# lan496/torch-m3gnet

Hardware: AMD Instinct MI355X
Metric: atom-steps/sec (energy+forces) on 10k-atom PBC batch, 1/2/4/8 MI355X (higher is better)
Workload: dtype f32; 1 GPU; single 10000-atom fcc Cu PBC supercell per GPU (10x10x25 cells, a=3.61 A, jitter 0.025 A), r_cut 5 A / 3-body 4 A, default M3GNet (l_max=n_max=3, D=64, 3 blocks), energy+forces+stress; precision=fp32, atoms_per_gpu=10000, edges_per_gpu=420000, triplets_per_gpu=3060000

## Files before the change

torch-m3gnet_amd/csrc/m3g_api.hip:

```cpp
#include <cmath>
#include <cstdarg>
#include <cstdio>
#include <cstdlib>
#include <cstring>

#include "m3g_internal.h"

namespace m3g {

static thread_local char g_err[512] = "";
void set_error(const char* fmt, ...) {
  va_list ap;
  va_start(ap, fmt);
  vsnprintf(g_err, sizeof(g_err), fmt, ap);
  va_end(ap);
}

static inline size_t align_up(size_t x, size_t a = 256) { return (x + a - 1) / a * a; }

static void layout_mlp(MlpW& m, size_t& off) {
  auto take = [&](size_t n) { size_t r = off; off += (n + 63) / 64 * 64; return r; };
  m.w1a_t = take(kDP * 2 * kDP); m.w1b_t = take(kDP * 2 * kDP); m.w1c_t = take(kDP * 2 * kDP);
  m.b1 = take(2 * kDP);
  m.w2d_t = take(kDP * kDP); m.w2g_t = take(kDP * kDP);
// ... 284 lines not shown
  return M3G_OK;
}

extern "C" int m3g_plan_set_const(m3g_plan* plan, const char* name, const float* host_data, int64_t numel) {
  if (!plan || !name || !host_data) { set_error("m3g_plan_set_const: null argument"); return M3G_ERR_VALUE; }
  auto exp = expected_consts(plan->cfg);
  auto it = exp.find(name);
  if (it == exp.end()) { set_error("unknown constant '%s'", name); return M3G_ERR_VALUE; }
  if (it->second != numel) { set_error("constant '%s': expected %lld values, got %lld", name, (long long)it->second, (long long)numel); return M3G_ERR_VALUE; }
  plan->cvals[name].assign(host_data, host_data + numel);
  plan->committed = false;
  return M3G_OK;
}

extern "C" int m3g_plan_set_option(m3g_plan* plan, const char* name, int32_t value) {
  if (!plan || !name) { set_error("m3g_plan_set_option: null argument"); return M3G_ERR_VALUE; }
  if (strcmp(name, "edge_kernel") == 0) {
    if (value < 0 || value > 2) { set_error("edge_kernel must be 0 (VALU baseline), 1 (MFMA) or 2 (any-size path)"); return M3G_ERR_VALUE; }
    if (plan->generic && value != 2) { set_error("this model size only runs on the any-size path (edge_kernel = 2)"); return M3G_ERR_UNSUPPORTED; }
    plan->edge_kernel = value;
    return M3G_OK;
  }
  if (strcmp(name, "precision") == 0) {
    if (value != kPrecF32 && value != kPrecBf16x3 && value != kPrecF16x3) {
      set_error("precision must be 0 (fp32: exact fp32 MFMA products), 1 (bf16x3 split products) or 2 (f16x3: scaled fp16 split products)");
      return M3G_ERR_VALUE;
    }
    plan->precision = value;
    return M3G_OK;
  }
  if (strcmp(name, "save_p1") == 0) {
    plan->save_p1 = value != 0;
    return M3G_OK;
  }
  if (strcmp(name, "save_p2") == 0) {
    plan->save_p2 = value != 0;
    return M3G_OK;
  }
  if (strcmp(name, "rev_kernel") == 0) {
    if (value != 0 && value != 1) { set_error("rev_kernel must be 0 (node-MLP + edge-MLP kernel pair) or 1 (fused)"); return M3G_ERR_VALUE; }
    plan->rev_kernel = value;
    return M3G_OK;
  }
  if (strcmp(name, "small_tiles") == 0) {
    if (value < 0) { set_error("small_tiles must be >= 0"); return M3G_ERR_VALUE; }
    plan->small_tiles = value;
    plan->small_tiles_fwd = value;
    drop_graphs(plan);
    return M3G_OK;
  }
  if (strcmp(name, "small_tiles_fwd") == 0) {
    if (value < 0) { set_error("small_tiles_fwd must be >= 0"); return M3G_ERR_VALUE; }
    plan->small_tiles_fwd = value;
    drop_graphs(plan);
    return M3G_OK;
  }
  if (strcmp(name, "dp1_by_dst") == 0) {
    plan->dp1_by_dst = value != 0;
    drop_graphs(plan);
    return M3G_OK;
  }
  if (strcmp(name, "split_node_tiles") == 0) {
    if (value < 0) { set_error("split_node_tiles must be >= 0"); return M3G_ERR_VALUE; }
    plan->split_node_tiles = value;
    drop_graphs(plan);
    return M3G_OK;
  }
  if (strcmp(name, "fuse_node_tb") == 0) {
    plan->fuse_node_tb = value != 0;
    drop_graphs(plan);
    return M3G_OK;
  }
  if (strcmp(name, "debug_node_tb_polls") == 0) {
    plan->debug_node_tb_polls = value;
    drop_graphs(plan);
    return M3G_OK;
  }
  if (strcmp(name, "split_tail") == 0) {
    if (value < 0 || value > 2) { set_error("split_tail must be 0 (never), 1 (a single left-over tile) or 2 (one or two)"); return M3G_ERR_VALUE; }
    plan->split_tail = value;
    drop_graphs(plan);
    return M3G_OK;
  }
  if (strcmp(name, "small_launches") == 0) {
    plan->small_launches = value != 0;
    drop_graphs(plan);
    return M3G_OK;
  }
  if (strcmp(name, "graph_replay") == 0) {
    plan->graph_replay = value != 0;
    if (!plan->graph_replay) drop_graphs(plan);
    return M3G_OK;
  }
  if (strcmp(name, "overlap") == 0) {
    plan->overlap = value != 0;
    return M3G_OK;
  }
  if (strcmp(name, "threebody_moments") == 0) {
    plan->tb_moments = value != 0;
    return M3G_OK;
  }
  if (strcmp(name, "legendre_backward") == 0) {
    if (value != 0 && value != 1) { set_error("legendre_backward: 0 (exact derivative) or 1 (the reference's backward)"); return M3G_ERR_VALUE; }
    plan->legendre_ref = value != 0;
    drop_graphs(plan);
    return M3G_OK;
  }
  if (strcmp(name, "readout_f16") == 0) {
    plan->readout_f16 = value != 0;
    return M3G_OK;
  }
  if (strcmp(name, "stress_mode") == 0) {
    if (value != 0 && value != 1) { set_error("stress_mode must be 0 (reference: sum pos (x) F / V) or 1 (pair virial)"); return M3G_ERR_VALUE; }
    plan->stress_mode = value;
    return M3G_OK;
  }
  if (strcmp(name, "debug_force_move") == 0) {
    plan->debug_force_move = value != 0;
    plan->committed = false;
    return M3G_OK;
  }
  if (strcmp(name, "stamps") == 0) {
    plan->stamp_target = value == 3 ? 2 : value == 2 ? 1 : 0;
    if (value && !plan->d_stamps) {
      M3G_HIP_CHECK(hipMalloc((void**)&plan->d_stamps, 256 * 16 * 12 * sizeof(unsigned long long)));
      M3G_HIP_CHECK(hipMemset(plan->d_stamps, 0, 256 * 16 * 12 * sizeof(unsigned long long)));
    } else if (!value && plan->d_stamps) {
      (void)hipFree(plan->d_stamps);
      plan->d_stamps = nullptr;
    }
    return M3G_OK;
  }
  set_error("unknown option '%s'", name);
  return M3G_ERR_VALUE;
}

extern "C" int m3g_debug_read_stamps(m3g_plan* plan, uint64_t* host_out ) {
  if (!plan || !host_out || !plan->d_stamps) { set_error("stamps not enabled"); return M3G_ERR_STATE; }
  M3G_HIP_CHECK(hipMemcpy(host_out, plan->d_stamps, 256 * 16 * 12 * sizeof(unsigned long long), hipMemcpyDeviceToHost));
  return M3G_OK;
}

extern "C" int m3g_plan_commit(m3g_plan* plan) {
  if (!plan) { set_error("m3g_plan_commit: null plan"); return M3G_ERR_VALUE; }
  drop_graphs(plan);
  const m3g_config& cfg = plan->cfg;
  for (auto& kv : expected_params(cfg))
    if (!plan->params.count(kv.first)) { set_error("parameter '%s' was never set", kv.first.c_str()); return M3G_ERR_STATE; }
  for (auto& kv : expected_consts(cfg))
    if (!plan->cvals.count(kv.first)) { set_error("constant '%s' was never set", kv.first.c_str()); return M3G_ERR_STATE; }
  const int D = cfg.embedding_dim, R = cfg.n_max, L = cfg.l_max, C = L * R, B = cfg.num_blocks;
  {
    int dev = 0;
    M3G_HIP_CHECK(hipGetDevice(&dev));
    if (plan->device >= 0 && (plan->device != dev || plan->debug_force_move)) {
      M3G_HIP_CHECK(hipSetDevice(plan->device));
      M3G_HIP_CHECK(hipDeviceSynchronize());
      if (plan->d_weights) { (void)hipFree(plan->d_weights); plan->d_weights = nullptr; }
      free_mfma_images(plan);
      generic_free(plan);
      if (plan->d_stamps) { (void)hipFree(plan->d_stamps); plan->d_stamps = nullptr; }
      release_device_handles(plan);
      M3G_HIP_CHECK(hipSetDevice(dev));
      plan->debug_force_move = false;
    }
    M3G_HIP_CHECK(hipDeviceSynchronize());
// ... 52 lines not shown
    put_t(blob, bw.tb_wd_t, kDP, wd, D, C, 0, C); put_t(blob, bw.tb_wg_t, kDP, wg, D, C, 0, C);
    put_n(blob, bw.tb_wd, kCP, wd, D, C, 0, C); put_n(blob, bw.tb_wg, kCP, wg, D, C, 0, C);
    pack_mlp(blob, bw.e, *plan, cv + ".concat_edge_update", cv + ".edge_linear.weight", D, R);
    pack_mlp(blob, bw.n, *plan, cv + ".concat_node_update", cv + ".node_linear.weight", D, R);
  }
  {
    const ReadoutW& r = wl.ro;
    snprintf(buf, sizeof buf, "model.%d.gated", 6 + 2 * B);
    std::string ro = buf;
    const float* wd0 = plan->params.at(ro + ".dense.0.weight").data();
    const float* wg0 = plan->params.at(ro + ".gate.0.weight").data();
    const float* wd2 = plan->params.at(ro + ".dense.2.weight").data();
    const float* wg2 = plan->params.at(ro + ".gate.2.weight").data();
    put_t(blob, r.w1d_t, kDP, wd0, D, D, 0, D); put_t(blob, r.w1g_t, kDP, wg0, D, D, 0, D);
    put_t(blob, r.w2d_t, kDP, wd2, D, D, 0, D); put_t(blob, r.w2g_t, kDP, wg2, D, D, 0, D);
    put_n(blob, r.w1d, kDP, wd0, D, D, 0, D); put_n(blob, r.w1g, kDP, wg0, D, D, 0, D);
    put_n(blob, r.w2d, kDP, wd2, D, D, 0, D); put_n(blob, r.w2g, kDP, wg2, D, D, 0, D);
    for (int o = 0; o < D; ++o) {
      blob[r.b1d + o] = plan->params.at(ro + ".dense.0.bias")[o];
      blob[r.b1g + o] = plan->params.at(ro + ".gate.0.bias")[o];
      blob[r.b2d + o] = plan->params.at(ro + ".dense.2.bias")[o];
      blob[r.b2g + o] = plan->params.at(ro + ".gate.2.bias")[o];
      blob[r.w3d + o] = plan->params.at(ro + ".dense.4.weight")[o];
      blob[r.w3g + o] = plan->params.at(ro + ".gate.4.weight")[o];
    }
    blob[r.b3] = plan->params.at(ro + ".dense.4.bias")[0];
    blob[r.b3 + 1] = plan->params.at(ro + ".gate.4.bias")[0];
  }
  if (!plan->d_weights) M3G_HIP_CHECK(hipMalloc((void**)&plan->d_weights, wl.total * sizeof(float)));
  M3G_HIP_CHECK(hipMemcpy(plan->d_weights, blob.data(), wl.total * sizeof(float), hipMemcpyHostToDevice));
  { int rc = pack_mfma_images(plan); if (rc) return rc; }
  plan->committed = true;
  return M3G_OK;
}

extern "C" int m3g_workspace_bytes(const m3g_plan* plan, int64_t N, int64_t E, int64_t T, int64_t S, size_t* bytes) {
  if (!plan || !bytes || N < 0 || E < 0 || T < 0 || S < 0) { set_error("m3g_workspace_bytes: bad argument"); return M3G_ERR_VALUE; }
  if (plan->edge_kernel == 2) { *bytes = generic_workspace_bytes(plan, N, E, T, S); return M3G_OK; }
  Consts c{};
  c.B = plan->cfg.num_blocks;
  *bytes = work_carve(c, plan->edge_kernel == 1, saved_activations(plan), N, E, T, S, nullptr).total_bytes;
  return M3G_OK;
}

static bool ensure_side_stream(const m3g_plan* plan) {
  if (plan->side_stream) return true;
  if (hipStreamCreateWithFlags(&plan->side_stream, hipStreamNonBlocking) != hipSuccess) { plan->side_stream = nullptr; return false; }
  if (hipEventCreateWithFlags(&plan->ev_fork, hipEventDisableTiming) != hipSuccess ||
      hipEventCreateWithFlags(&plan->ev_join, hipEventDisableTiming) != hipSuccess)
    return false;
  return true;
}

static void drop_graphs(const m3g_plan* plan) {
  for (auto& g : plan->graphs) {
    if (g.exec) (void)hipGraphExecDestroy(g.exec);
    if (g.graph) (void)hipGraphDestroy(g.graph);
  }
  plan->graphs.clear();
}

static int energy_forces_graph(const m3g_plan* plan, const m3g_io* io, void* workspace, size_t workspace_bytes, hipStream_t caller) {
  hipStream_t s = caller;
  const bool via_side = caller == nullptr;
  if (via_side) {
    if (!ensure_side_stream(plan)) { set_error("graph_replay: could not create the internal stream"); return M3G_ERR_HIP; }
    s = plan->side_stream;
    M3G_HIP_CHECK(hipEventRecord(plan->ev_fork, caller));
    M3G_HIP_CHECK(hipStreamWaitEvent(s, plan->ev_fork, 0));
  }
  auto join = [&]() -> int {
    if (via_side) {
      M3G_HIP_CHECK(hipEventRecord(plan->ev_join, s));
      M3G_HIP_CHECK(hipStreamWaitEvent(caller, plan->ev_join, 0));
    }
    return M3G_OK;
  };
  std::vector<unsigned char> key(sizeof(m3g_io) + sizeof(void*) * 2 + sizeof(size_t) + 4 * sizeof(int));
  unsigned char* k = key.data();
  memcpy(k, io, sizeof(m3g_io)); k += sizeof(m3g_io);
  memcpy(k, &workspace, sizeof(void*)); k += sizeof(void*);
  memcpy(k, &s, sizeof(void*)); k += sizeof(void*);
  memcpy(k, &workspace_bytes, sizeof(size_t)); k += sizeof(size_t);
  const int opts[4] = {plan->edge_kernel, plan->rev_kernel + 2 * plan->save_p1 + 4 * plan->save_p2 + 8 * plan->tb_moments + 16 * plan->precision + 64 * plan->readout_f16, plan->stress_mode, plan->overlap};
  memcpy(k, opts, sizeof(opts));
  for (auto& g : plan->graphs)
    if (g.key == key) { M3G_HIP_CHECK(hipGraphLaunch(g.exec, s)); return join(); }
  if (plan->graphs.size() >= 8) drop_graphs(plan);
  m3g_plan::GraphEntry ge;
  ge.key = key;
  M3G_HIP_CHECK(hipStreamBeginCapture(s, hipStreamCaptureModeThreadLocal));
  plan->capturing = true;
  const int rc = m3g_energy_forces(plan, io, workspace, workspace_bytes, (void*)s);
  plan->capturing = false;
  hipError_t e = hipStreamEndCapture(s, &ge.graph);
  if (rc != M3G_OK) { if (ge.graph) (void)hipGraphDestroy(ge.graph); return rc; }
  if (e != hipSuccess || !ge.graph) { set_error("hipStreamEndCapture failed: %s", hipGetErrorString(e)); return M3G_ERR_HIP; }
  e = hipGraphInstantiate(&ge.exec, ge.graph, nullptr, nullptr, 0);
  if (e != hipSuccess) { (void)hipGraphDestroy(ge.graph); set_error("hipGraphInstantiate failed: %s", hipGetErrorString(e)); return M3G_ERR_HIP; }
  plan->graphs.push_back(ge);
  M3G_HIP_CHECK(hipGraphLaunch(ge.exec, s));
  return join();
}

extern "C" int m3g_count_launches(const m3g_plan* plan, const m3g_io* io, void* workspace, size_t workspace_bytes, int32_t* kernel_launches,
                                  int32_t* other_operations) {
  if (!plan || !io || !kernel_launches) { set_error("m3g_count_launches: null argument"); return M3G_ERR_VALUE; }
  if (plan->capturing) { set_error("m3g_count_launches: a capture is in progress"); return M3G_ERR_STATE; }
  hipStream_t s = nullptr;
  M3G_HIP_CHECK(hipStreamCreateWithFlags(&s, hipStreamNonBlocking));
  hipGraph_t graph = nullptr;
  hipError_t e = hipStreamBeginCapture(s, hipStreamCaptureModeThreadLocal);
  if (e != hipSuccess) { (void)hipStreamDestroy(s); set_error("hipStreamBeginCapture failed: %s", hipGetErrorString(e)); return M3G_ERR_HIP; }
  const bool profile = plan->profile;
  plan->capturing = true;
  plan->profile = false;
  const int rc = m3g_energy_forces(plan, io, workspace, workspace_bytes, (void*)s);
  plan->capturing = false;
  plan->profile = profile;
  e = hipStreamEndCapture(s, &graph);
  (void)hipStreamDestroy(s);
  if (rc != M3G_OK) { if (graph) (void)hipGraphDestroy(graph); return rc; }
  if (e != hipSuccess || !graph) { set_error("hipStreamEndCapture failed: %s", hipGetErrorString(e)); return M3G_ERR_HIP; }
  size_t n = 0;
  e = hipGraphGetNodes(graph, nullptr, &n);
  std::vector<hipGraphNode_t> nodes(n);
  if (e == hipSuccess && n) e = hipGraphGetNodes(graph, nodes.data(), &n);
  int kernels = 0, other = 0;
  for (size_t i = 0; e == hipSuccess && i < n; ++i) {
    hipGraphNodeType ty;
    e = hipGraphNodeGetType(nodes[i], &ty);
    if (e != hipSuccess) break;
    if (ty == hipGraphNodeTypeKernel) ++kernels;
    else if (ty != hipGraphNodeTypeEmpty) ++other;
  }
  (void)hipGraphDestroy(graph);
  if (e != hipSuccess) { set_error("m3g_count_launches: reading the captured graph failed: %s", hipGetErrorString(e)); return M3G_ERR_HIP; }
  *kernel_launches = kernels;
  if (other_operations) *other_operations = other;
  return M3G_OK;
}

static int dp1_format(const m3g_plan* plan) {
  if (!fused_reverse(plan)) return kDp1F32;
  if (dp1_rows_by_dst(plan)) return kDp1F32ByDst;
  return plan->precision == kPrecBf16x3 ? kDp1Packed : plan->precision == kPrecF16x3 ? kDp1Fixed : kDp1F32;
}

extern "C" int m3g_energy_forces(const m3g_plan* plan, const m3g_io* io, void* workspace, size_t workspace_bytes,
                                 void* stream_) {
  if (!plan || !io) { set_error("m3g_energy_forces: null argument"); return M3G_ERR_VALUE; }
  if (!plan->committed) { set_error("m3g_energy_forces: plan parameters not committed"); return M3G_ERR_STATE; }
  {
    int dev = -1;
    M3G_HIP_CHECK(hipGetDevice(&dev));
    if (dev != plan->device) {
      set_error("m3g_energy_forces: the plan was committed on device %d but the current device is %d (commit again on this device)", plan->device, dev);
      return M3G_ERR_STATE;
    }
  }
  if (plan->graph_replay && !plan->capturing && !plan->profile && !plan->overlap)
    return energy_forces_graph(plan, io, workspace, workspace_bytes, (hipStream_t)stream_);
  const int64_t N = io->n_atoms, E = io->n_edges, T = io->n_triplets, S = io->n_structs;
  if (N < 0 || E < 0 || T < 0 || S < 0) { set_error("negative size"); return M3G_ERR_VALUE; }
  if (!io->total_energy || !io->topo || (N > 0 && (!io->pos || !io->atom_types)) || (S > 0 && !io->lattice) ||
      (E > 0 && !io->edge_cell_shift)) {
    set_error("m3g_energy_forces: missing required pointer");
// ... 202 lines not shown
```

torch-m3gnet_amd/csrc/m3g_edge_common.h:

```cpp
#pragma once
#include <utility>

#include "m3g_device.h"
#include "m3g_internal.h"
#include "m3g_dual_chain.h"
#include "m3g_dual_f32.h"
#include "m3g_mfma_common.h"

namespace m3g {

constexpr int kFwdLdsFloats = 8 * kTbSteps * 64 + 2 * (8 * 4 * 4 * 64 + 2 * (4 * 4 * 4 * 64) + 2 * 4 * 64 + 4 * 64) + 4 * 64;
constexpr int kRevMlpFloats = 8 * 4 * 4 * 64 + 4 * (4 * 4 * 4 * 64) + 2 * 4 * 64 + 4 * 8 * 4 * 64 + 64 * 4;
constexpr int kRevEdgeFloats = kRevMlpFloats + 8 * kTbSteps * 64 + 8 * 4 * 64;
#ifndef M3G_WAVES_FWD
#define M3G_WAVES_FWD 16
#endif
constexpr int kWaves = M3G_WAVES_FWD;
#ifndef M3G_WAVES_FWD_H
#define M3G_WAVES_FWD_H 12
#endif
template <int PREC>
#ifndef M3G_WAVES_FWD_BF
#define M3G_WAVES_FWD_BF 12
#endif
// ... 329 lines not shown
struct TbIn { float mb[TBS]; };
template <int TBS>
struct TbIn<kPrecF16x3, TBS> { f16x8 hi, lo; float inv; };

template <int PREC, int TBS>
__device__ __forceinline__ TbIn<PREC, TBS> tb_load(const float* __restrict__ m, int arow, int q, float w_inv) {
  TbIn<PREC, TBS> r;
  if constexpr (PREC == kPrecF16x3) {
    f32x4 v[2] = {f32x4{0.f, 0.f, 0.f, 0.f}, f32x4{0.f, 0.f, 0.f, 0.f}};
    if (arow >= 0 && q < 2) {
      const float* row = m + (int64_t)arow * kCP + 8 * q;
      v[0] = *(const f32x4*)row;
      v[1] = *(const f32x4*)(row + 4);
    }
    const EdgeScale sc = edge_scale<2>(v);
    split8h(v[0], v[1], sc.s, r.hi, r.lo);
    r.inv = sc.inv * w_inv;
  } else {
    static_for<TBS>([&]<int s>() { r.mb[s] = arow >= 0 ? m[(int64_t)arow * kCP + 4 * s + q] : 0.f; });
  }
  return r;
}
template <int PREC, int TBS>
__device__ __forceinline__ void tb_preact_p(const float* tbimg, const TbIn<PREC, TBS>& in, f32x4 (&p)[8], int lane) {
  if constexpr (PREC == kPrecF16x3) {
    const f16x8* hi = reinterpret_cast<const f16x8*>(tbimg) + (lane & 31);
    const f16x8* lo = hi + 8 * 32;
    f16x8 ah = hi[0], al = lo[0];
    static_for<8>([&]<int ob>() {
      f16x8 nh = ah, nl = al;
      if constexpr (ob + 1 < 8) { nh = hi[(ob + 1) * 32]; nl = lo[(ob + 1) * 32]; }
#ifndef M3G_NO_FWD_CHAIN_PREFETCH
      __builtin_amdgcn_sched_barrier(0);
#endif
      f32x4 t = {0.f, 0.f, 0.f, 0.f};
      t = mfma_f16(ah, in.hi, t);
      t = mfma_f16(ah, in.lo, t);
      t = mfma_f16(al, in.hi, t);
      p[ob] = t * in.inv;
#ifndef M3G_NO_FWD_CHAIN_PREFETCH
      __builtin_amdgcn_sched_barrier(0);
#endif
      ah = nh; al = nl;
    });
  } else {
    tb_preact<TBS>(tbimg, in.mb, p, lane);
  }
}

__device__ __forceinline__ void gather_tables(const float* __restrict__ TA, const float* __restrict__ TB, int mlp, int64_t ci,
                                              int64_t cj, int qd, f32x4 (&p1)[8]) {
#ifdef M3G_DIAG_NO_GATHER
  static_for<8>([&]<int ob>() { p1[ob] = f32x4{0.1f, 0.2f, 0.3f, 0.4f}; });
  return;
#endif
  const float* ta = TA + ci * (4 * kDP) + mlp * (2 * kDP) + 4 * qd;
  const float* tb = TB + cj * (4 * kDP) + mlp * (2 * kDP) + 4 * qd;
  static_for<8>([&]<int ob>() { p1[ob] = *(const f32x4*)(ta + ob * 16) + *(const f32x4*)(tb + ob * 16); });
}

struct RevArgs {
  int64_t E, tiles;
  const float* img;
  const int32_t *src, *dst;
  const float *h, *m, *dx_new;
  const int32_t* act_id;
  const float *TA, *TB;
  const float* e_tile;
  const float* e2_tile;
  float* de_soa;
  float* dcn;
  int de_is_zero;
  float* dm;
  float* dh;
  float* dp1;
  unsigned long long* stamps;
  float *seg_head, *seg_first;
  const float* p1;
  const float* p2;
  float w_inv;
  float* dp1_scale;
  const int32_t* in_pos;
  int split_tail;
};

__device__ __forceinline__ float sum_lane_quarters(float x) {
  const unsigned u = __builtin_bit_cast(unsigned, x);
  auto r16 = __builtin_amdgcn_permlane16_swap(u, u, false, false);
  const float y = __builtin_bit_cast(float, (unsigned)r16[0]) + __builtin_bit_cast(float, (unsigned)r16[1]);
  const unsigned v = __builtin_bit_cast(unsigned, y);
  auto r32 = __builtin_amdgcn_permlane32_swap(v, v, false, false);
  return __builtin_bit_cast(float, (unsigned)r32[0]) + __builtin_bit_cast(float, (unsigned)r32[1]);
}

__device__ __forceinline__ void store_dh(float* dh, int64_t edge, int64_t E, f32x4 dhv, int qd) {
  static_for<4>([&]<int rr>() { dhv[rr] = sum_lane_quarters(dhv[rr]); });
  if (qd == 0 && edge < E) *(f32x4*)(dh + edge * kRP) = dhv;
}

inline int grid_for_tiles(int64_t tiles, int  = kWaves) {
#ifdef M3G_GRID_PACKED
  int64_t wgs = (tiles + kWaves - 1) / kWaves;
#else
  int64_t wgs = tiles;
#endif
  wgs = (wgs + 7) / 8 * 8;
  if (wgs < 8) wgs = 8;
  if (wgs > 256) wgs = 256;
  return (int)wgs;
}

inline int tb_steps_for(int C) { return (C + 3) / 4; }
inline int64_t tiles_for(int64_t E) { return (E + kTileEdges - 1) / kTileEdges; }

#define M3G_TBS_SWITCH(C_, CALL)                     \
  switch (tb_steps_for(C_)) {                        \
    case 1: { constexpr int TBS = 1; CALL; } break;  \
    case 2: { constexpr int TBS = 2; CALL; } break;  \
    case 3: { constexpr int TBS = 3; CALL; } break;  \
    default: { constexpr int TBS = 4; CALL; } break; \
  }

#define M3G_PREC_SWITCH(P_, CALL)                                            \
  if ((P_) == kPrecF32) { constexpr int PREC = kPrecF32; CALL; }             \
  else if ((P_) == kPrecF16x3) { constexpr int PREC = kPrecF16x3; CALL; }    \
  else { constexpr int PREC = kPrecBf16x3; CALL; }

}
```

torch-m3gnet_amd/csrc/m3g_edge_rev_f32.hip:

```cpp
#include "m3g_edge_common.h"
#include "m3g_edge_split_rev.h"

namespace m3g {

MfmaRevF32Layout mfma_rev_f32_layout() {
  MfmaRevF32Layout L{};
  int off = 0;
  auto take = [&](int n) { int r = off; off += n; return r; };
  L.tb = take(8 * kTbSteps * 64);
  L.tbT = take(1 * 32 * 64);
  for (int m = 0; m < 2; ++m) {
    L.mlp[m].w2d = take(64 * 64);
    L.mlp[m].w2g = take(64 * 64);
    L.mlp[m].w1cT = take(4 * 32 * 64);
    L.mlp[m].b2 = take(2 * 4 * 64);
    L.mlp[m].wl = take(64 * 4);
    L.mlp[m].wld = take(4 * 64);
  }
  L.adj = take(4 * 64);
  L.adjp = take(64 * 4);
  L.total = off;
  return L;
}

// ... 22 lines not shown
    bias_step<4, 0>(lds + L.b2, d2, lane);
    bias_step<4, 4>(lds + L.b2 + 4 * 64, d2, lane);
    static_for<2>([&]<int half>() {
      f32x4 hid[4];
      static_for<4>([&]<int ob>() {
        static_for<4>([&]<int r>() {
          const float p = p1[4 * half + ob][r], sg = fsigmoid(p);
          hid[ob][r] = p * sg;
          p1[4 * half + ob][r] = sg * (1.f + p * (1.f - sg));
        });
      });
      chain_dual32<4, 0, 4 * half>(lds + (half == 0 ? L.w2d : L.w2g), hid, d2, lane);
      M3G_F32_FENCE();
    });
  }
  const float hb_sel = qd == 0 ? hv[0] : qd == 1 ? hv[1] : qd == 2 ? hv[2] : hv[3];
  static_for<4>([&]<int ob>() {
    const f32x4 sl = mfma16(lds[L.wld + ob * 64 + lane], hb_sel, f32x4{0.f, 0.f, 0.f, 0.f});
#ifndef M3G_F32_SCALAR_ACT
    static_for<2>([&]<int k>() {
      const f32x2 p2d = {d2[ob][2 * k], d2[ob][2 * k + 1]}, p2g = {d2[4 + ob][2 * k], d2[4 + ob][2 * k + 1]};
      const f32x2 du = {d_upd[ob][2 * k], d_upd[ob][2 * k + 1]}, s_lin = {sl[2 * k], sl[2 * k + 1]};
      f32x2 sd, dsd;
      silu_pair(p2d, sd, dsd);
      const f32x2 sg = sigmoid_pair(p2g);
      const f32x2 a_g = du * sg;
      const f32x2 d_s = a_g * sd;
      const f32x2 d_o = a_g * s_lin;
      const f32x2 dd = d_o * dsd;
      const f32x2 dgt = (d_s * s_lin) * (1.f - sg);
      const f32x4 w0 = *(const f32x4*)(lds + L.wl + (ob * 16 + 4 * qd + 2 * k) * 4);
      const f32x4 w1 = *(const f32x4*)(lds + L.wl + (ob * 16 + 4 * qd + 2 * k + 1) * 4);
      f32x2 h01 = {dhv[0], dhv[1]}, h23 = {dhv[2], dhv[3]};
      h01 += f32x2{w0[0], w0[1]} * d_s[0]; h23 += f32x2{w0[2], w0[3]} * d_s[0];
      h01 += f32x2{w1[0], w1[1]} * d_s[1]; h23 += f32x2{w1[2], w1[3]} * d_s[1];
      dhv[0] = h01[0]; dhv[1] = h01[1]; dhv[2] = h23[0]; dhv[3] = h23[1];
      d2[ob][2 * k] = dd[0]; d2[ob][2 * k + 1] = dd[1];
      d2[4 + ob][2 * k] = dgt[0]; d2[4 + ob][2 * k + 1] = dgt[1];
    });
#else
    static_for<4>([&]<int r>() {
      const float p2d = d2[ob][r], p2g = d2[4 + ob][r];
      const f32x4 w = *(const f32x4*)(lds + L.wl + (ob * 16 + 4 * qd + r) * 4);
      const float s_lin = sl[r];
      const float sg = fsigmoid(p2g), sgd = fsigmoid(p2d), sd = p2d * sgd;
      const float du = d_upd[ob][r];
      const float d_out = du * s_lin, d_s = du * sd * sg;
      dhv[0] += d_s * w[0]; dhv[1] += d_s * w[1]; dhv[2] += d_s * w[2]; dhv[3] += d_s * w[3];
      d2[ob][r] = d_out * sg * (sgd * (1.f + p2d * (1.f - sgd)));
      d2[4 + ob][r] = d_out * sd * sg * (1.f - sg);
    });
#endif
    asm volatile("" : "+v"(dhv[0]), "+v"(dhv[1]), "+v"(dhv[2]), "+v"(dhv[3]));
  });
  zero(contrib);
  M3G_F32_FENCE();
  static_for<2>([&]<int half>() {
    f32x4 dp1[4];
    zero(dp1);
    f32x4 ds1[4];
    if constexpr (SAVED_P2) static_for<4>([&]<int ob>() { ds1[ob] = load_tile4(p1_src + (4 * half + ob) * 256); });
    chain_dual32_t<4, 4 * half, 0>(lds + (half == 0 ? L.w2d : L.w2g), d2, dp1, lane);
    if constexpr (SAVED_P2) static_for<4>([&]<int ob>() { dp1[ob] *= ds1[ob]; });
    else static_for<4>([&]<int ob>() { dp1[ob] *= p1[4 * half + ob]; });
    if (NEED_DP1 && edge < a.E) {
      float* row = a.dp1 + drow * (4 * kDP) + MLP * (2 * kDP) + half * kDP + 4 * qd;
      static_for<4>([&]<int ob>() { *(f32x4*)(row + ob * 16) = dp1[ob]; });
    }
    chain_f32<4, 4, 0, 0, 8, 4 * half>(lds + L.w1cT, dp1, contrib, lane);
    if (NEED_DP1) {
      if (edge >= a.E) zero(dp1);
      seg_scan(dp1, sk);
      seg_store<MLP * 8 + 4 * half>(dp1, sk, a.seg_head, a.seg_first, tile, ci, qd);
    }
    M3G_F32_FENCE();
  });
}

__device__ __forceinline__ void load_p2(const RevArgs& a, int64_t tile, int mlp, f32x4 (&d2)[8]) {
  const float* src = a.p2 + tile * (2 * kP1TileFloats) + mlp * kP1TileFloats + (threadIdx.x & 63) * 4;
  static_for<8>([&]<int ob>() { d2[ob] = load_tile4(src + ob * 256); });
}

template <int TBS, bool NEED_DP1, int WAVES, bool SAVED_P2>
__global__ void __launch_bounds__(64 * WAVES) k_edge_rev_f32(RevArgs a, MfmaRevF32Layout L) {
  __shared__ __attribute__((aligned(16))) float lds[kRevF32Floats + 4];
  int* q_head = reinterpret_cast<int*>(lds + kRevF32Floats);
  load_image(lds, a.img, kRevF32Floats, q_head);
  const int lane = threadIdx.x & 63, qd = lane >> 4;
  TileQueue queue(a.tiles, q_head);
  int tail = 0;
  if constexpr (SAVED_P2 && WAVES == 8) tail = (queue.count & 3) >= 1 && (queue.count & 3) <= a.split_tail ? (queue.count & 3) : 0;
  const int count_a = queue.count - tail;
  const int wave_id = __builtin_amdgcn_readfirstlane((int)(threadIdx.x >> 6));
  int ticket = queue.fetch(lane);
  int ci_i = 0, cj_i;
  if (ticket < count_a) load_ends(a.src, nullptr, queue.base + ticket, a.E, lane, ci_i, cj_i);
  constexpr bool FIRST = !NEED_DP1;
  while (ticket < count_a) {
    const int64_t tile = queue.base + ticket;
    ticket = queue.fetch(lane);
    const bool has_next = ticket < count_a;
    int nci = 0, ncj = 0;
    if (has_next) load_ends(a.src, nullptr, queue.base + ticket, a.E, lane, nci, ncj);
    int lv = lane;
    asm volatile("" : "+v"(lv));
    const int64_t edge = tile * kTileEdges + (lane & 15);
    const int64_t ec = edge < a.E ? edge : a.E - 1;
    const int64_t ci = ci_i;
    const int64_t drow = (NEED_DP1 && a.in_pos) ? (int64_t)a.in_pos[ec] : edge;
    const SegMasks sk = seg_masks((int)ci, lane);
    float* de_tile = a.de_soa + tile * kTileFloats + lane * 4;
    const f32x4 hv = *(const f32x4*)(a.h + ec * kRP);
    f32x4 dhv = {0.f, 0.f, 0.f, 0.f};
    float mb[TBS];
    const int arow = a.act_id[ec];
    static_for<TBS>([&]<int s>() { mb[s] = arow >= 0 ? a.m[(int64_t)arow * kCP + 4 * s + qd] : 0.f; });
    f32x4 de[4], contrib[4], d2e[8];
    {
      f32x4 dmsg[4];
      const float* xrow = a.dx_new + ci * kDP + 4 * qd;
      static_for<4>([&]<int blk>() { dmsg[blk] = *(const f32x4*)(xrow + blk * 16); });
      f32x4 d2n[8];
      if constexpr (SAVED_P2) load_p2(a, tile, 1, d2n);
#ifdef M3G_P2_PREFETCH
      if constexpr (SAVED_P2) load_p2(a, tile, 0, d2e);
#endif
      mlp_reverse_f32<NEED_DP1, 1, SAVED_P2>(lds, L.mlp[1], a, edge, drow, tile, ci, sk, hv, dmsg, contrib, dhv, lv, d2n);
    }
    if (a.de_is_zero) {
      static_for<4>([&]<int blk>() { de[blk] = contrib[blk]; });
    } else {
      static_for<4>([&]<int blk>() { de[blk] = load_tile4(de_tile + blk * 256) + contrib[blk]; });
    }
    asm volatile("" : "+v"(lv));
    M3G_F32_FENCE();
#ifndef M3G_P2_PREFETCH
    if constexpr (SAVED_P2) load_p2(a, tile, 0, d2e);
#endif
    mlp_reverse_f32<NEED_DP1, 0, SAVED_P2>(lds, L.mlp[0], a, edge, drow, tile, ci, sk, hv, de, contrib, dhv, lv, d2e);
    static_for<4>([&]<int blk>() {
      de[blk] += contrib[blk];
      if (!FIRST) *(f32x4*)(de_tile + blk * 256) = de[blk];
    });
    if (FIRST) {
      const float hb = qd == 0 ? hv[0] : qd == 1 ? hv[1] : qd == 2 ? hv[2] : hv[3];
      static_for<4>([&]<int blk>() {
        const f32x4 pe = mfma16(lds[L.adj + blk * 64 + lv], hb, f32x4{0.f, 0.f, 0.f, 0.f});
        static_for<4>([&]<int r>() {
          const f32x4 w = *(const f32x4*)(lds + L.adjp + (blk * 16 + 4 * qd + r) * 4);
          const float t = de[blk][r] * fdsilu(pe[r]);
          dhv[0] += t * w[0]; dhv[1] += t * w[1]; dhv[2] += t * w[2]; dhv[3] += t * w[3];
        });
        asm volatile("" : "+v"(dhv[0]), "+v"(dhv[1]), "+v"(dhv[2]), "+v"(dhv[3]));
      });
    }
    f32x4 d8[8];
    tb_preact<TBS>(lds + L.tb, mb, d8, lv);
#ifndef M3G_F32_SCALAR_ACT
    static_for<4>([&]<int blk>() {
      static_for<2>([&]<int k>() {
        f32x2 sd, dsd;
        silu_pair(f32x2{d8[blk][2 * k], d8[blk][2 * k + 1]}, sd, dsd);
        const f32x2 sg = sigmoid_pair(f32x2{d8[4 + blk][2 * k], d8[4 + blk][2 * k + 1]});
        const f32x2 a_g = f32x2{de[blk][2 * k], de[blk][2 * k + 1]} * sg;
        const f32x2 dd = a_g * dsd, dgt = (a_g * sd) * (1.f - sg);
        d8[blk][2 * k] = dd[0]; d8[blk][2 * k + 1] = dd[1];
        d8[4 + blk][2 * k] = dgt[0]; d8[4 + blk][2 * k + 1] = dgt[1];
      });
    });
#else
    static_for<4>([&]<int blk>() {
      static_for<4>([&]<int r>() {
        const float p = d8[blk][r], sgd = fsigmoid(p), sg = fsigmoid(d8[4 + blk][r]);
        d8[blk][r] = de[blk][r] * sg * (sgd * (1.f + p * (1.f - sgd)));
        d8[4 + blk][r] = de[blk][r] * (p * sgd) * sg * (1.f - sg);
      });
    });
#endif
    f32x4 dmv[1];
    zero(dmv);
    chain_f32<1, 8>(lds + L.tbT, d8, dmv, lv);
    store_dh(a.dh, edge, a.E, dhv, qd);
    if (edge < a.E && arow >= 0) *(f32x4*)(a.dm + (int64_t)arow * kCP + 4 * qd) = dmv[0];
    ci_i = nci;
  }
  if constexpr (SAVED_P2 && WAVES == 8) {
    if (tail) {
      rev_split_run<TBS, NEED_DP1>(a, L, lds , lds, 2, wave_id >> 2, wave_id & 3, lane,
                                   queue.base + count_a + (wave_id >> 2), queue.base + queue.count, 2);
    }
  }
}

void launch_edge_rev_f32(const m3g_plan* plan, const Consts& c, const Topo& t, const Work& w, int b, const float* dx_new,
                         bool de_is_zero, hipStream_t s) {
  const int64_t tiles = tiles_for(t.E);
  if (tiles == 0) return;
  if (tiles <= plan->small_tiles && launch_edge_rev_split(plan, c, t, w, b, dx_new, de_is_zero, s)) return;
  const MfmaRevF32Layout L = mfma_rev_f32_layout();
  static_assert(kRevF32Floats * 4 + 16 <= 160 * 1024, "fused fp32 reverse image exceeds the LDS");
  const float* img = plan->d_mfma_revf32 + (size_t)b * L.total;
  RevArgs ar{t.E, tiles, img, t.src, t.dst, w.h, w.m[b], dx_new, t.act_id, nullptr, nullptr, nullptr, nullptr, w.de_soa, nullptr,
             de_is_zero ? 1 : 0, w.dm, w.dh_parts + (size_t)b * t.E * kRP, w.dp1, nullptr, w.seg_head, w.seg_first, w.p1_blk[b],
             saves_p2(plan) ? w.p2_blk[b] : nullptr, 1.f, nullptr, dp1_rows_by_dst(plan) ? t.in_pos : nullptr, plan->split_tail};
  static_assert(2 * kRevSplitGroupFloats + kRevSplitTabFloats <= kRevF32Floats, "the split tail's exchange buffers must fit in the image's LDS");
  constexpr int WV = kWavesRevF32;
  dim3 grid(grid_for_tiles(tiles, WV)), block(64 * WV);
  const bool p2 = saves_p2(plan);
#define M3G_REV_F32_LAUNCH(NEED, P2) M3G_TBS_SWITCH(c.C, hipLaunchKernelGGL((k_edge_rev_f32<TBS, NEED, WV, P2>), grid, block, 0, s, ar, L))
  if (b > 0) { if (p2) { M3G_REV_F32_LAUNCH(true, true); } else { M3G_REV_F32_LAUNCH(true, false); } }
  else { if (p2) { M3G_REV_F32_LAUNCH(false, true); } else { M3G_REV_F32_LAUNCH(false, false); } }
#undef M3G_REV_F32_LAUNCH
}

}
```

torch-m3gnet_amd/csrc/m3g_internal.h:

```cpp
#pragma once
#include <hip/hip_runtime.h>

#include <cstddef>
#include <cstdint>
#include <map>
#include <string>
#include <vector>

#include "../../include/m3gnet_hip.h"

namespace m3g {

constexpr int kDP = 64;
constexpr int kLCap = 4;
constexpr int kRCap = 4;
constexpr int kCP = 16;
constexpr int kRP = 4;
constexpr int kMaxBlocks = 8;
constexpr int kPrecF32 = 0;
constexpr int kPrecBf16x3 = 1;
constexpr int kPrecF16x3 = 2;
constexpr int kNumPrec = 3;

void set_error(const char* fmt, ...);
// ... 88 lines not shown
struct MfmaMlpFused {
  int w1c;
  int w2d, w2g;
  int b2;
  int wl;
  int wld;
};
struct MfmaRevFusedLayout {
  int tb;
  int tbT;
  MfmaMlpFused mlp[2];
  int adj;
  int adjp;
  int total;
};
struct MfmaMlpRevF32 {
  int w2d, w2g;
  int w1cT;
  int b2;
  int wl;
  int wld;
};
struct MfmaRevF32Layout {
  int tb;
  int tbT;
  MfmaMlpRevF32 mlp[2];
  int adj;
  int adjp;
  int total;
};
MfmaRevF32Layout mfma_rev_f32_layout();
constexpr int kNodeRowBlocks = 33;
constexpr int kNodeImgFloats = kNodeRowBlocks * 16 * 64 + kNodeRowBlocks * 16;
struct ReadoutImg {
  static constexpr int w1 = 0;
  static constexpr int w2d = w1 + 8 * 2 * 512;
  static constexpr int w2g = w2d + 4 * 2 * 512;
  static constexpr int w2dT = w2g + 4 * 2 * 512;
  static constexpr int w2gT = w2dT + 4 * 2 * 512;
  static constexpr int w1T = w2gT + 4 * 2 * 512;
  static constexpr int b1 = w1T + 4 * 4 * 512;
  static constexpr int b2 = b1 + 128;
  static constexpr int w3 = b2 + 128;
  static constexpr int b3 = w3 + 128;
  static constexpr int total = b3 + 4;
};
MfmaFwdLayout mfma_fwd_layout();
MfmaRevLayout mfma_rev_layout();
MfmaRevFusedLayout mfma_rev_fused_layout();

}

struct m3g_plan {
  m3g_config cfg;
  m3g::Consts consts;
  m3g::WeightLayout wl;
  std::map<std::string, std::vector<float>> params;
  std::map<std::string, std::vector<float>> cvals;
  float* d_weights = nullptr;
  float* d_mfma_fwd[m3g::kNumPrec] = {nullptr, nullptr, nullptr};
  float* d_mfma_rev[m3g::kNumPrec] = {nullptr, nullptr, nullptr};
  float* d_mfma_revf = nullptr;
  float* d_mfma_revf_h = nullptr;
  float* d_mfma_revf32 = nullptr;
  float* d_node_img[m3g::kNumPrec] = {nullptr, nullptr, nullptr};
  int precision = m3g::kPrecF32;
  float w_scale_inv = 1.f;
  int save_p1 = 1;
  int save_p2 = 1;
  int device = -1;
  bool generic = false;
  float* d_generic = nullptr;
  std::map<std::string, size_t> generic_off;
  float* d_readout_img = nullptr;
  float* d_readout_img_h = nullptr;
  float ro_w_scale_inv = 1.f;
  int small_tiles_fwd = 3072;
  int small_tiles = 1536;
  int dp1_by_dst = 0;
  int split_node_tiles = 128;
  int fuse_node_tb = 1;
  int debug_node_tb_polls = 0;
  int split_tail = 1;
  int small_launches = 1;
  int rev_kernel = 1;
  bool readout_f16 = false;
  bool legendre_ref = false;
  bool tb_moments = true;
  int stress_mode = 0;
  int edge_kernel = 1;
  int stamp_target = 0;
  unsigned long long* d_stamps = nullptr;
  bool committed = false;
  bool debug_force_move = false;
  mutable hipStream_t side_stream = nullptr;
  mutable hipEvent_t ev_fork = nullptr, ev_join = nullptr;
  int overlap = 0;
  int graph_replay = 0;
  struct GraphEntry { std::vector<unsigned char> key; hipGraph_t graph = nullptr; hipGraphExec_t exec = nullptr; };
  mutable std::vector<GraphEntry> graphs;
  mutable bool capturing = false;
  mutable bool profile = false;
  mutable std::vector<hipEvent_t> ev_pool;
  mutable std::vector<int> ev_stage;
  mutable size_t ev_used = 0;
};

namespace m3g {

#define M3G_DISPATCH_LR(L_, R_, BODY)                         \
  switch ((L_) * 8 + (R_)) {                                  \
    case 1 * 8 + 1: { constexpr int L = 1, R = 1; BODY; } break; \
    case 1 * 8 + 2: { constexpr int L = 1, R = 2; BODY; } break; \
    case 1 * 8 + 3: { constexpr int L = 1, R = 3; BODY; } break; \
    case 1 * 8 + 4: { constexpr int L = 1, R = 4; BODY; } break; \
    case 2 * 8 + 1: { constexpr int L = 2, R = 1; BODY; } break; \
    case 2 * 8 + 2: { constexpr int L = 2, R = 2; BODY; } break; \
    case 2 * 8 + 3: { constexpr int L = 2, R = 3; BODY; } break; \
    case 2 * 8 + 4: { constexpr int L = 2, R = 4; BODY; } break; \
    case 3 * 8 + 1: { constexpr int L = 3, R = 1; BODY; } break; \
    case 3 * 8 + 2: { constexpr int L = 3, R = 2; BODY; } break; \
    case 3 * 8 + 3: { constexpr int L = 3, R = 3; BODY; } break; \
    case 3 * 8 + 4: { constexpr int L = 3, R = 4; BODY; } break; \
    case 4 * 8 + 1: { constexpr int L = 4, R = 1; BODY; } break; \
    case 4 * 8 + 2: { constexpr int L = 4, R = 2; BODY; } break; \
    case 4 * 8 + 3: { constexpr int L = 4, R = 3; BODY; } break; \
    case 4 * 8 + 4: { constexpr int L = 4, R = 4; BODY; } break; \
    default: break;                                           \
  }

#ifndef M3G_TB_ROWS
#define M3G_TB_ROWS 128
#endif
constexpr int kTbRows = M3G_TB_ROWS;
#ifndef M3G_TB_CAP
#define M3G_TB_CAP 255
#endif
constexpr int kTbCap = M3G_TB_CAP;
constexpr int kTbListShort = 32, kTbListLong = 96;
constexpr int kTopoFlags = 16;
constexpr int kTbFastAtoms = 64;
constexpr int kTbCapShort = kTbRows + 64 < kTbCap ? kTbRows + 64 : kTbCap;
struct Topo {
  int64_t N, E, T, S;
  int32_t* src;
  int32_t* dst;
  int32_t* row_ptr;
  int32_t* in_ptr;
  int32_t* in_edge;
  int32_t* in_pos;
  int32_t* in_pair;
  int32_t* t1_ptr;
  int32_t* t1_e2;
  int32_t* t2_ptr;
  int32_t* t2_e1;
  int32_t* act_list;
  int32_t* act_scan;
  int32_t* act_id;
  int32_t* arow_ptr;
  int32_t* t1_e2c;
  int32_t* t2_e1c;
  uint8_t* t1_b;
  uint8_t* t2_b;
  int32_t* act_dst;
  int32_t* tb_win;
  int32_t* tb_fast;
// ... 141 lines not shown
```

Baseline: 4.162 million atom-steps/s.

## Run reverse three-body gate pass only over active-edge rows per block

Adds a tb_active_only mode (on by default) to the fused fp32 reverse edge kernel. Instead of running the three-body gate backward and its matmul chain on every edge tile, the main loop only records the range of active-edge rows each block touched. After a block-wide reduction, a second loop processes just those active rows from act_list, with software prefetch of the next tile. This is meant to skip MFMA and activation work on edges that fall outside the 3-body cutoff. In exchange it adds a __syncthreads, extra LDS for the per-wave bounds, and a second pass that re-reads m and de from global memory.

```diff
diff --git a/torch-m3gnet_amd/csrc/m3g_api.hip b/torch-m3gnet_amd/csrc/m3g_api.hip
--- a/torch-m3gnet_amd/csrc/m3g_api.hip
+++ b/torch-m3gnet_amd/csrc/m3g_api.hip
@@ -390,6 +390,12 @@
     drop_graphs(plan);
     return M3G_OK;
   }
+  if (strcmp(name, "tb_active_only") == 0) {
+    if (value < 0 || value > 1) { set_error("tb_active_only must be 0 or 1"); return M3G_ERR_VALUE; }
+    plan->tb_active_only = value;
+    drop_graphs(plan);
+    return M3G_OK;
+  }
   if (strcmp(name, "small_launches") == 0) {
     plan->small_launches = value != 0;
     drop_graphs(plan);
@@ -608,7 +614,7 @@
   memcpy(k, &workspace, sizeof(void*)); k += sizeof(void*);
   memcpy(k, &s, sizeof(void*)); k += sizeof(void*);
   memcpy(k, &workspace_bytes, sizeof(size_t)); k += sizeof(size_t);
-  const int opts[4] = {plan->edge_kernel, plan->rev_kernel + 2 * plan->save_p1 + 4 * plan->save_p2 + 8 * plan->tb_moments + 16 * plan->precision + 64 * plan->readout_f16, plan->stress_mode, plan->overlap};
+  const int opts[4] = {plan->edge_kernel, plan->rev_kernel + 2 * plan->save_p1 + 4 * plan->save_p2 + 8 * plan->tb_moments + 16 * plan->precision + 64 * plan->readout_f16 + 128 * plan->tb_active_only, plan->stress_mode, plan->overlap};
   memcpy(k, opts, sizeof(opts));
   for (auto& g : plan->graphs)
     if (g.key == key) { M3G_HIP_CHECK(hipGraphLaunch(g.exec, s)); return join(); }
diff --git a/torch-m3gnet_amd/csrc/m3g_edge_common.h b/torch-m3gnet_amd/csrc/m3g_edge_common.h
--- a/torch-m3gnet_amd/csrc/m3g_edge_common.h
+++ b/torch-m3gnet_amd/csrc/m3g_edge_common.h
@@ -435,6 +435,7 @@
   float* dp1_scale;
   const int32_t* in_pos;
   int split_tail;
+  const int32_t* act_list;
 };
 
 __device__ __forceinline__ float sum_lane_quarters(float x) {
diff --git a/torch-m3gnet_amd/csrc/m3g_edge_rev_f32.hip b/torch-m3gnet_amd/csrc/m3g_edge_rev_f32.hip
--- a/torch-m3gnet_amd/csrc/m3g_edge_rev_f32.hip
+++ b/torch-m3gnet_amd/csrc/m3g_edge_rev_f32.hip
@@ -128,9 +128,99 @@
   static_for<8>([&]<int ob>() { d2[ob] = load_tile4(src + ob * 256); });
 }
 
-template <int TBS, bool NEED_DP1, int WAVES, bool SAVED_P2>
+__device__ __forceinline__ void tb_rev_gates(const f32x4 (&de)[4], f32x4 (&d8)[8]) {
+#ifndef M3G_F32_SCALAR_ACT
+  static_for<4>([&]<int blk>() {
+    static_for<2>([&]<int k>() {
+      f32x2 sd, dsd;
+      silu_pair(f32x2{d8[blk][2 * k], d8[blk][2 * k + 1]}, sd, dsd);
+      const f32x2 sg = sigmoid_pair(f32x2{d8[4 + blk][2 * k], d8[4 + blk][2 * k + 1]});
+      const f32x2 a_g = f32x2{de[blk][2 * k], de[blk][2 * k + 1]} * sg;
+      const f32x2 dd = a_g * dsd, dgt = (a_g * sd) * (1.f - sg);
+      d8[blk][2 * k] = dd[0]; d8[blk][2 * k + 1] = dd[1];
+      d8[4 + blk][2 * k] = dgt[0]; d8[4 + blk][2 * k + 1] = dgt[1];
+    });
+  });
+#else
+  static_for<4>([&]<int blk>() {
+    static_for<4>([&]<int r>() {
+      const float p = d8[blk][r], sgd = fsigmoid(p), sg = fsigmoid(d8[4 + blk][r]);
+      d8[blk][r] = de[blk][r] * sg * (sgd * (1.f + p * (1.f - sgd)));
+      d8[4 + blk][r] = de[blk][r] * (p * sgd) * sg * (1.f - sg);
+    });
+  });
+#endif
+}
+
+template <int TBS>
+struct TbActRow {
+  int row;
+  bool valid;
+  float mb[TBS];
+  f32x4 de[4];
+};
+template <int TBS>
+__device__ __forceinline__ void tb_act_load(const RevArgs& a, int row, int edge, bool valid, int qd, TbActRow<TBS>& t) {
+  t.row = row;
+  t.valid = valid;
+  const int64_t rr = valid ? row : 0, ee = valid ? edge : 0;
+  static_for<TBS>([&]<int s>() { t.mb[s] = valid ? a.m[rr * kCP + 4 * s + qd] : 0.f; });
+  const float* src = a.de_soa + (ee / kTileEdges) * kTileFloats + ((ee % kTileEdges) + 16 * qd) * 4;
+  static_for<4>([&]<int blk>() { t.de[blk] = valid ? *(const f32x4*)(src + blk * 256) : f32x4{0.f, 0.f, 0.f, 0.f}; });
+}
+
+template <int TBS>
+__device__ __forceinline__ void tb_rev_active(const RevArgs& a, const float* lds, const MfmaRevF32Layout& L, int rlo, int rhi, int64_t e_lo,
+                                              int64_t e_hi, int wave_id, int waves, int lane) {
+  const int qd = lane >> 4;
+  const int n_tiles = rhi >= rlo ? (rhi - rlo) / kTileEdges + 1 : 0;
+  auto row_of = [&](int t) { return rlo + t * kTileEdges + (lane & 15); };
+  auto edge_of = [&](int t) { const int row = row_of(t); return t < n_tiles && row <= rhi ? a.act_list[row] : -1; };
+  auto valid_of = [&](int t, int edge) {
+    return row_of(t) <= rhi && edge >= e_lo && edge < e_hi;
+  };
+  int t = wave_id;
+  if (t >= n_tiles) return;
+  int edge = edge_of(t), edge_n = edge_of(t + waves);
+  TbActRow<TBS> cur;
+  tb_act_load<TBS>(a, row_of(t), edge, valid_of(t, edge), qd, cur);
+  for (;;) {
+    const int tn = t + waves;
+    const bool has_next = tn < n_tiles;
+    TbActRow<TBS> nxt;
+    int edge_nn = -1;
+    if (has_next) {
+      tb_act_load<TBS>(a, row_of(tn), edge_n, valid_of(tn, edge_n), qd, nxt);
+      edge_nn = edge_of(tn + waves);
+    }
+    int lv = lane;
+    asm volatile("" : "+v"(lv));
+    f32x4 d8[8];
+    tb_preact<TBS>(lds + L.tb, cur.mb, d8, lv);
+    tb_rev_gates(cur.de, d8);
+    f32x4 dmv[1];
+    zero(dmv);
+    chain_f32<1, 8>(lds + L.tbT, d8, dmv, lv);
+    if (cur.valid) *(f32x4*)(a.dm + (int64_t)cur.row * kCP + 4 * qd) = dmv[0];
+    if (!has_next) break;
+    cur = nxt;
+    edge_n = edge_nn;
+    t = tn;
+  }
+}
+
+__device__ __forceinline__ int wave_min_i(int v) {
+  static_for<6>([&]<int k>() { v = min(v, __shfl_xor(v, 1 << k)); });
+  return v;
+}
+__device__ __forceinline__ int wave_max_i(int v) {
+  static_for<6>([&]<int k>() { v = max(v, __shfl_xor(v, 1 << k)); });
+  return v;
+}
+
+template <int TBS, bool NEED_DP1, int WAVES, bool SAVED_P2, bool TBA>
 __global__ void __launch_bounds__(64 * WAVES) k_edge_rev_f32(RevArgs a, MfmaRevF32Layout L) {
-  __shared__ __attribute__((aligned(16))) float lds[kRevF32Floats + 4];
+  __shared__ __attribute__((aligned(16))) float lds[kRevF32Floats + 4 + 2 * WAVES];
   int* q_head = reinterpret_cast<int*>(lds + kRevF32Floats);
   load_image(lds, a.img, kRevF32Floats, q_head);
   const int lane = threadIdx.x & 63, qd = lane >> 4;
@@ -143,6 +233,7 @@
   int ci_i = 0, cj_i;
   if (ticket < count_a) load_ends(a.src, nullptr, queue.base + ticket, a.E, lane, ci_i, cj_i);
   constexpr bool FIRST = !NEED_DP1;
+  int rlo = INT_MAX, rhi = -1;
   while (ticket < count_a) {
     const int64_t tile = queue.base + ticket;
     ticket = queue.fetch(lane);
@@ -201,35 +292,31 @@
         asm volatile("" : "+v"(dhv[0]), "+v"(dhv[1]), "+v"(dhv[2]), "+v"(dhv[3]));
       });
     }
-    f32x4 d8[8];
-    tb_preact<TBS>(lds + L.tb, mb, d8, lv);
-#ifndef M3G_F32_SCALAR_ACT
-    static_for<4>([&]<int blk>() {
-      static_for<2>([&]<int k>() {
-        f32x2 sd, dsd;
-        silu_pair(f32x2{d8[blk][2 * k], d8[blk][2 * k + 1]}, sd, dsd);
-        const f32x2 sg = sigmoid_pair(f32x2{d8[4 + blk][2 * k], d8[4 + blk][2 * k + 1]});
-        const f32x2 a_g = f32x2{de[blk][2 * k], de[blk][2 * k + 1]} * sg;
-        const f32x2 dd = a_g * dsd, dgt = (a_g * sd) * (1.f - sg);
-        d8[blk][2 * k] = dd[0]; d8[blk][2 * k + 1] = dd[1];
-        d8[4 + blk][2 * k] = dgt[0]; d8[4 + blk][2 * k + 1] = dgt[1];
-      });
-    });
-#else
-    static_for<4>([&]<int blk>() {
-      static_for<4>([&]<int r>() {
-        const float p = d8[blk][r], sgd = fsigmoid(p), sg = fsigmoid(d8[4 + blk][r]);
-        d8[blk][r] = de[blk][r] * sg * (sgd * (1.f + p * (1.f - sgd)));
-        d8[4 + blk][r] = de[blk][r] * (p * sgd) * sg * (1.f - sg);
-      });
-    });
-#endif
-    f32x4 dmv[1];
-    zero(dmv);
-    chain_f32<1, 8>(lds + L.tbT, d8, dmv, lv);
-    store_dh(a.dh, edge, a.E, dhv, qd);
-    if (edge < a.E && arow >= 0) *(f32x4*)(a.dm + (int64_t)arow * kCP + 4 * qd) = dmv[0];
+    if constexpr (!TBA) {
+      f32x4 d8[8];
+      tb_preact<TBS>(lds + L.tb, mb, d8, lv);
+      tb_rev_gates(de, d8);
+      f32x4 dmv[1];
+      zero(dmv);
+      chain_f32<1, 8>(lds + L.tbT, d8, dmv, lv);
+      store_dh(a.dh, edge, a.E, dhv, qd);
+      if (edge < a.E && arow >= 0) *(f32x4*)(a.dm + (int64_t)arow * kCP + 4 * qd) = dmv[0];
+    } else {
+      if (FIRST && edge < a.E && arow >= 0) static_for<4>([&]<int blk>() { *(f32x4*)(de_tile + blk * 256) = de[blk]; });
+      store_dh(a.dh, edge, a.E, dhv, qd);
+      if (edge < a.E && arow >= 0) { rlo = min(rlo, arow); rhi = max(rhi, arow); }
+    }
     ci_i = nci;
+  }
+  if constexpr (TBA) {
+    int* bounds = reinterpret_cast<int*>(lds + kRevF32Floats + 4);
+    rlo = wave_min_i(rlo);
+    rhi = wave_max_i(rhi);
+    if (lane == 0) { bounds[2 * wave_id] = rlo; bounds[2 * wave_id + 1] = rhi; }
+    __syncthreads();
+    static_for<WAVES>([&]<int wv>() { rlo = min(rlo, bounds[2 * wv]); rhi = max(rhi, bounds[2 * wv + 1]); });
+    const int64_t e_lo = queue.base * kTileEdges, e_hi = (queue.base + count_a) * kTileEdges;
+    tb_rev_active<TBS>(a, lds, L, rlo, rhi, e_lo, e_hi < a.E ? e_hi : a.E, wave_id, WAVES, lane);
   }
   if constexpr (SAVED_P2 && WAVES == 8) {
     if (tail) {
@@ -245,18 +332,19 @@
   if (tiles == 0) return;
   if (tiles <= plan->small_tiles && launch_edge_rev_split(plan, c, t, w, b, dx_new, de_is_zero, s)) return;
   const MfmaRevF32Layout L = mfma_rev_f32_layout();
-  static_assert(kRevF32Floats * 4 + 16 <= 160 * 1024, "fused fp32 reverse image exceeds the LDS");
+  static_assert(kRevF32Floats * 4 + 16 + 2 * kWavesRevF32 * 4 <= 160 * 1024, "fused fp32 reverse image exceeds the LDS");
   const float* img = plan->d_mfma_revf32 + (size_t)b * L.total;
   RevArgs ar{t.E, tiles, img, t.src, t.dst, w.h, w.m[b], dx_new, t.act_id, nullptr, nullptr, nullptr, nullptr, w.de_soa, nullptr,
              de_is_zero ? 1 : 0, w.dm, w.dh_parts + (size_t)b * t.E * kRP, w.dp1, nullptr, w.seg_head, w.seg_first, w.p1_blk[b],
-             saves_p2(plan) ? w.p2_blk[b] : nullptr, 1.f, nullptr, dp1_rows_by_dst(plan) ? t.in_pos : nullptr, plan->split_tail};
+             saves_p2(plan) ? w.p2_blk[b] : nullptr, 1.f, nullptr, dp1_rows_by_dst(plan) ? t.in_pos : nullptr, plan->split_tail, t.act_list};
   static_assert(2 * kRevSplitGroupFloats + kRevSplitTabFloats <= kRevF32Floats, "the split tail's exchange buffers must fit in the image's LDS");
   constexpr int WV = kWavesRevF32;
   dim3 grid(grid_for_tiles(tiles, WV)), block(64 * WV);
   const bool p2 = saves_p2(plan);
-#define M3G_REV_F32_LAUNCH(NEED, P2) M3G_TBS_SWITCH(c.C, hipLaunchKernelGGL((k_edge_rev_f32<TBS, NEED, WV, P2>), grid, block, 0, s, ar, L))
-  if (b > 0) { if (p2) { M3G_REV_F32_LAUNCH(true, true); } else { M3G_REV_F32_LAUNCH(true, false); } }
-  else { if (p2) { M3G_REV_F32_LAUNCH(false, true); } else { M3G_REV_F32_LAUNCH(false, false); } }
+  const bool tba = plan->tb_active_only != 0 && t.act_list != nullptr;
+#define M3G_REV_F32_LAUNCH(NEED, P2, TBA) M3G_TBS_SWITCH(c.C, hipLaunchKernelGGL((k_edge_rev_f32<TBS, NEED, WV, P2, TBA>), grid, block, 0, s, ar, L))
+  if (b > 0) { if (p2 && tba) { M3G_REV_F32_LAUNCH(true, true, true); } else if (p2) { M3G_REV_F32_LAUNCH(true, true, false); } else { M3G_REV_F32_LAUNCH(true, false, false); } }
+  else { if (p2 && tba) { M3G_REV_F32_LAUNCH(false, true, true); } else if (p2) { M3G_REV_F32_LAUNCH(false, true, false); } else { M3G_REV_F32_LAUNCH(false, false, false); } }
 #undef M3G_REV_F32_LAUNCH
 }
 
diff --git a/torch-m3gnet_amd/csrc/m3g_internal.h b/torch-m3gnet_amd/csrc/m3g_internal.h
--- a/torch-m3gnet_amd/csrc/m3g_internal.h
+++ b/torch-m3gnet_amd/csrc/m3g_internal.h
@@ -194,6 +194,7 @@
   int fuse_node_tb = 1;
   int debug_node_tb_polls = 0;
   int split_tail = 1;
+  int tb_active_only = 1;
   int small_launches = 1;
   int rev_kernel = 1;
   bool readout_f16 = false;
```

Result: no change. 4.153 million atom-steps/s (median of 3 runs) (-0.2%).
